# zju3dv/Mirror-NeRF

Hardware: AMD Instinct MI355X
Metric: rendered rays/sec (primary+reflected) (higher is better)
Workload: dtype f32 carried as hi/lo f16 pairs (f16 MFMA, f32 accumulate; max |diff| to the fp32 chain 3e-6)

## Files before the change

include/mnrf.h:

```cpp
#ifndef MNRF_H
#define MNRF_H

#include <stdint.h>

#ifdef __cplusplus
extern "C" {
#endif

#define MNRF_OK 0
#define MNRF_ERR_ARG (-1)
#define MNRF_ERR_LAUNCH (-2)
#define MNRF_ERR_UNSUPPORTED (-3)

#define MNRF_N_PARAMS 32

#define MNRF_SIGMA_ONLY 1u
#define MNRF_GRAD_NORMAL 2u
#define MNRF_SPLIT_F16 4u

#define MNRF_TCNN_GRAD_F16 16u
#define MNRF_TCNN_GRAD_FIXED 512u
#define MNRF_TCNN_F16 256u
#define MNRF_TCNN_TABLE_F16 1024u
#define MNRF_TCNN_VALU 8u
// ... 6 lines not shown

#define MNRF_GUARD_SATURATED 1u
#define MNRF_GUARD_WEIGHT 2u
#define MNRF_GUARD_IN_FORWARD 128u
#define MNRF_GUARD_IN_BACKWARD 256u
#define MNRF_GUARD_IN_SECOND_ORDER 512u
#define MNRF_GUARD_ENC_RANGE 4u

const char* mnrf_last_error(void);
int mnrf_version(void);

int64_t mnrf_packed_floats(void);

int mnrf_pack_weights(const float* const* params, float* packed, void* stream);
int mnrf_pack_weights_n(int n_models, const float* const* params, float* const* packed, void* stream);

int mnrf_embed(const float* x, int64_t n, int c, int n_freqs, float* out, void* stream);

int mnrf_field_forward(float* packed, unsigned flags, int64_t B,
                       const float* xyz, int64_t xyz_stride,
                       const float* rays, const float* z_vals, int spr,
                       const float* dir_emb, int64_t dir_stride,
                       float* sigma, float* rgb, float* pred_normal, float* is_mirror,
                       float* normal, float* geo_feat, void* stream);

int mnrf_sample_coarse(const float* rays, int64_t n_rays, const float* z_steps, int n_samples,
                       int use_disp, float perturb, const float* perturb_rand, float* z_vals,
                       void* stream);

int mnrf_composite(const float* rays, int64_t n_rays, int S, const float* sigma, const float* z_vals,
// ... 308 lines not shown
```

mirror_nerf_amd/_lib.py:

```python
import ctypes
import os
import subprocess

import torch

_HERE = os.path.dirname(os.path.abspath(__file__))
LIB_PATH = os.environ.get("MNRF_LIB", os.path.join(_HERE, "libmnrf_hip.so"))
CSRC = os.path.join(_HERE, "csrc")

_c_f = ctypes.c_void_p
_c_i = ctypes.c_void_p
_i64 = ctypes.c_int64
_int = ctypes.c_int
_u32 = ctypes.c_uint
_flt = ctypes.c_float
_str = ctypes.c_void_p

MNRF_SIGMA_ONLY = 1
MNRF_GRAD_NORMAL = 2
MNRF_SPLIT_F16 = 4
MNRF_TCNN_VALU = 8
MNRF_TCNN_F16 = 256
MNRF_TCNN_GRAD_FIXED = 512
MNRF_TCNN_TABLE_F16 = 1024
# ... 1 lines not shown
MNRF_CUT_MIRROR_HEAD = 64
MNRF_DW_ACCUMULATE = 128
MNRF_TRAIN_PLANES = 256
MNRF_PLANES_Y_HALF = 0x100000
MNRF_TCNN_GRAD_F16 = 16
MNRF_DETACH_W_MASK = 1
MNRF_DETACH_W_NORMAL = 2
N_PARAMS = 32

SIGNATURES = {
    "mnrf_last_error": (ctypes.c_char_p, []),
    "mnrf_version": (_int, []),
    "mnrf_packed_floats": (_i64, []),
    "mnrf_pack_weights": (_int, [ctypes.POINTER(ctypes.c_void_p), _c_f, _str]),
    "mnrf_pack_weights_n": (_int, [_int, ctypes.POINTER(ctypes.c_void_p), ctypes.POINTER(ctypes.c_void_p), _str]),
    "mnrf_embed": (_int, [_c_f, _i64, _int, _int, _c_f, _str]),
    "mnrf_field_forward": (_int, [_c_f, _u32, _i64, _c_f, _i64, _c_f, _c_f, _int, _c_f, _i64,
                                  _c_f, _c_f, _c_f, _c_f, _c_f, _c_f, _str]),
    "mnrf_sample_coarse": (_int, [_c_f, _i64, _c_f, _int, _int, _flt, _c_f, _c_f, _str]),
    "mnrf_composite": (_int, [_c_f, _i64, _int, _c_f, _c_f, _c_f, _c_f, _c_f, _c_f, _c_f, _int,
                              _c_f, _c_f, _c_f, _c_f, _c_f, _c_f, _c_f, _c_f, _c_f, _str]),
    "mnrf_composite_backward": (_int, [_c_f, _i64, _int] + [_c_f] * 7 + [_int] + [_c_f] * 17 + [_int, _c_f, _str]),
    "mnrf_reflect_backward": (_int, [_c_f, _c_f, _c_i, _i64, _c_f, _i64, _c_f, _c_f, _c_f, _str]),
    "mnrf_blend_backward": (_int, [_c_f, _c_f, _c_i, _i64, _i64, _int, _c_f, _c_f, _str]),
    "mnrf_embed_backward": (_int, [_c_f, _c_f, _i64, _int, _int, _c_f, _str]),
    "mnrf_ray_grads": (_int, [_c_f, _c_f, _c_f, _i64, _int, _c_f, _c_f, _str]),
    "mnrf_train_save_floats": (_i64, [_i64]),
    "mnrf_train_mask_words": (_i64, [_i64]),
    "mnrf_train_workspace_floats": (_i64, [_i64]),
    "mnrf_field_forward_train": (_int, [_c_f, _i64, _c_f, _i64, _c_f, _c_f, _int, _c_f, _i64] + [_c_f] * 9 + [_u32, _str]),
# ... 147 lines not shown
```

mirror_nerf_amd/csrc/mnrf_field.hip:

```cpp
#include <hip/hip_runtime.h>
#include <stdint.h>
#include <stdlib.h>

#include "mnrf_layout.h"
#include "mnrf_field_args.h"

namespace mnrf {

extern __shared__ __attribute__((aligned(16))) char smem[];

namespace s2 {
constexpr int S = 2;
constexpr int MIN_WAVES_PER_SIMD = 1;
constexpr int CHUNK_TILES = 16;
#include "mnrf_field_impl.inc"
#include "mnrf_field_bwd.inc"
}
namespace s1 {
constexpr int S = 1;
constexpr int MIN_WAVES_PER_SIMD = 2;
constexpr int CHUNK_TILES = 16;
#include "mnrf_field_impl.inc"
}

// ... 98 lines not shown
        const int nb = n_models - m0 < PACK_BATCH ? n_models - m0 : PACK_BATCH;
        PackBatch PB{};
        float* images[PACK_BATCH] = {};
        for (int m = 0; m < nb; ++m) {
            for (int i = 0; i < MNRF_N_PARAMS; ++i) PB.m[m].params[i] = params[(m0 + m) * MNRF_N_PARAMS + i];
            PB.m[m].packed = images[m] = packed[m0 + m];
        }
        hipLaunchKernelGGL(pack_kernel, dim3(blocks, nb), dim3(threads), 0, (hipStream_t)stream, PB, T);
        launch_split_pack(images, nb, (hipStream_t)stream);
        if (split32_enabled())
            for (int m = 0; m < nb; ++m) launch_split32_pack(params + (m0 + m) * MNRF_N_PARAMS, images[m], (hipStream_t)stream);
    }
    return mnrf_check_launch("mnrf_pack_weights");
}

extern "C" int mnrf_pack_weights(const float* const* params, float* packed, void* stream) {
    if (!params || !packed) return mnrf_fail(MNRF_ERR_ARG, "mnrf_pack_weights: null pointer");
    return mnrf_pack_weights_n(1, params, &packed, stream);
}

extern "C" int mnrf_field_forward(float* packed, unsigned flags, int64_t B, const float* xyz,
                                  int64_t xyz_stride, const float* rays, const float* z_vals, int spr,
                                  const float* dir_emb, int64_t dir_stride, float* sigma, float* rgb,
                                  float* pred_normal, float* is_mirror, float* normal, float* geo_feat,
                                  void* stream) {
    if (!packed) return mnrf_fail(MNRF_ERR_ARG, "mnrf_field_forward: packed weights are null");
    if (B < 0) return mnrf_fail(MNRF_ERR_ARG, "mnrf_field_forward: negative sample count");
    if (B == 0) return MNRF_OK;
    const bool sigma_only = flags & MNRF_SIGMA_ONLY;
    const bool grad = flags & MNRF_GRAD_NORMAL;
// ... 3 lines not shown
    if (!xyz && B % spr != 0) return mnrf_fail(MNRF_ERR_ARG, "mnrf_field_forward: B not a multiple of spr");
    if (!sigma_only && !dir_emb) return mnrf_fail(MNRF_ERR_ARG, "mnrf_field_forward: dir_emb required unless SIGMA_ONLY");
    if (grad && !normal) return mnrf_fail(MNRF_ERR_ARG, "mnrf_field_forward: GRAD_NORMAL needs the normal output");
    FieldArgs A{packed, flags, (long long)B, xyz, (long long)xyz_stride, rays, z_vals, spr, dir_emb,
                (long long)dir_stride, sigma, rgb, pred_normal, is_mirror, normal, geo_feat};
    static const int forced = [] {
        const char* e = getenv("MNRF_FIELD_VARIANT");
        if (e && e[0] == 's' && (e[1] == '1' || e[1] == '2')) return e[1] - '0';
        if (e && e[0] == 'h') return e[1] == 'x' ? 5 : (e[1] == '2' ? 4 : 3);
        return 0;
    }();
    const int variant = forced ? forced : ((flags & MNRF_SPLIT_F16) ? 3 + (int)((flags >> 3) & 3u) : (grad ? 1 : 2));
    const int rc = variant >= 3 ? launch_split(A, sigma_only, grad, variant - 3, (hipStream_t)stream)
                 : variant == 1 ? s1::launch(A, sigma_only, grad, (hipStream_t)stream)
                                : s2::launch(A, sigma_only, grad, (hipStream_t)stream);
    if (rc != 0) return mnrf_fail(MNRF_ERR_ARG, "mnrf_field_forward: too many samples for one launch");
    return mnrf_check_launch("mnrf_field_forward");
}

extern "C" int mnrf_fused_samples_per_ray(void) { return split48_ray_samples(); }

extern "C" int mnrf_field_composite_fused(float* packed, int64_t n_rays, const float* rays, const float* z_vals,
                                          const float* dir_emb, int64_t dir_stride, int white_back,
                                          float* weights, float* opacity, float* rgb_map, float* depth, float* mirror_mask,
                                          float* surf_normal, float* x_surface, void* stream) {
    if (!packed || !rays || !z_vals || !dir_emb) return mnrf_fail(MNRF_ERR_ARG, "mnrf_field_composite_fused: null pointer");
    if (n_rays < 0) return mnrf_fail(MNRF_ERR_ARG, "mnrf_field_composite_fused: negative ray count");
    if (n_rays == 0) return MNRF_OK;
    if (!split48_enabled() || split32_enabled())
        return mnrf_fail(MNRF_ERR_UNSUPPORTED, "mnrf_field_composite_fused: needs the 48-samples-per-wave tuning (MNRF_SPLIT48 != 0, MNRF_SPLIT32 unset)");
// ... 273 lines not shown
```

mirror_nerf_amd/csrc/mnrf_field_args.h:

```cpp
#pragma once
#include <hip/hip_runtime.h>
#include <stdint.h>

#include "../../include/mnrf.h"
#include "mnrf_layout.h"
#include "mnrf_dwp.h"

namespace mnrf {

typedef float f32x4 __attribute__((ext_vector_type(4)));

struct FieldArgs {
    const float* packed;
    unsigned flags;
    long long B;
    const float* xyz;
    long long xyz_stride;
    const float* rays;
    const float* z_vals;
    int spr;
    const float* dir_emb;
    long long dir_stride;
    float* sigma;
    float* rgb;
// ... 40 lines not shown
    const float* xyz; long long xyz_stride; const float* rays; const float* z_vals; int spr;
    const float* g_normal;
    const float* normal;
    const float* save_invj;
    const unsigned long long* save_mask;
    float* so;
    float* d_xyz;
    char* x2_planes;
    char* y2_planes;
    const unsigned* jmax;
    const int* n_live;
};

int launch_split(const FieldArgs& A, bool sigma_only, bool grad, int variant, hipStream_t s);
void launch_split_pack(float* const* packed, int n_images, hipStream_t s);
int launch_split_bwd(const FieldBwdArgs& A, hipStream_t s);
bool split48_enabled();
int launch_split48(const FieldArgs& A, bool sigma_only, hipStream_t s);
int split48_ray_samples();
bool split32_enabled();
int launch_split32(const FieldArgs& A, bool sigma_only, hipStream_t s);
void launch_split32_pack(const float* const* params, float* packed, hipStream_t s);
int launch_split_bwd2(const FieldBwd2Args& A, hipStream_t s);

}
```

mirror_nerf_amd/csrc/mnrf_field_split.hip:

```cpp
#include <hip/hip_runtime.h>
#include <stdint.h>
#include <type_traits>
#include <stdlib.h>

#include "mnrf_layout.h"
#include "mnrf_field_args.h"

namespace mnrf {

extern __shared__ __attribute__((aligned(16))) char smem[];

namespace h2 {
constexpr int S = 2;
constexpr int MIN_WAVES_PER_SIMD = 1;
constexpr int CHUNK_PAIRS = 8;
constexpr int RING_SLOTS = 4;
#include "mnrf_field_split.inc"
}
namespace h2x {
constexpr int S = 2;
constexpr int MIN_WAVES_PER_SIMD = 1;
constexpr int CHUNK_PAIRS = 16;
constexpr int RING_SLOTS = 3;
#include "mnrf_field_split.inc"
// ... 4 lines not shown
constexpr int S = 1;
constexpr int MIN_WAVES_PER_SIMD = 2;
constexpr int CHUNK_PAIRS = 8;
constexpr int RING_SLOTS = 3;
#define MNRF_SPLIT_NO_GRAD
#include "mnrf_field_split.inc"
#undef MNRF_SPLIT_NO_GRAD
}
#endif

int launch_split(const FieldArgs& A, bool sigma_only, bool grad, int variant, hipStream_t s) {
#ifdef MNRF_EXP_H1
    if (variant == 3 && !grad) return h1::launch(A, sigma_only, grad, s);
#endif
    if (!grad && variant == 0 && split32_enabled()) return launch_split32(A, sigma_only, s);
    if (!grad && variant == 0 && !A.geo_feat && split48_enabled()) return launch_split48(A, sigma_only, s);
    const bool big = variant == 0 ? grad : variant == 2;
    return big ? h2x::launch(A, sigma_only, grad, s) : h2::launch(A, sigma_only, grad, s);
}

int launch_split_bwd(const FieldBwdArgs& A, hipStream_t s) { return h2x::launch_bwd(A, s); }
int launch_split_bwd2(const FieldBwd2Args& A, hipStream_t s) { return h2x::launch_bwd2(A, s); }

struct SplitPackImages {
    float* packed[4];
};
__global__ void split_pack_kernel(SplitPackImages I, PartTable T) {
    float* packed = I.packed[blockIdx.y];
    const long long q = (long long)blockIdx.x * blockDim.x + threadIdx.x;
    constexpr long long FWD_LANES = (long long)SPLIT_FWD_PAIRS * 64;
// ... 52 lines not shown
    if (bad) atomicOr((unsigned*)(packed + PACKED_FLOATS - 1), MNRF_GUARD_WEIGHT);
    char* dst = (char*)(packed + (region == 2 ? OFF_SPLIT_HBWD : (region == 1 ? OFF_SPLIT_BWD : OFF_SPLIT_FWD))) + (long long)pair * PAIR_BYTES + lane * 16;
    *(h8v*)dst = hi;
    *(h8v*)(dst + PAIR_BYTES / 2) = lo;
}

void launch_split_pack(float* const* packed, int n_images, hipStream_t s) {
    PartTable T;
    build_parts(T);
    SplitPackImages I{};
    for (int m = 0; m < n_images; ++m) I.packed[m] = packed[m];
    const long long n = (long long)(SPLIT_FWD_PAIRS + SPLIT_BWD_PAIRS + SPLIT_HBWD_PAIRS) * 64;
    hipLaunchKernelGGL(split_pack_kernel, dim3((unsigned)((n + 255) / 256), n_images), dim3(256), 0, s, I, T);
}

}
```

mirror_nerf_amd/csrc/mnrf_field_split.inc:

```
constexpr int CHUNK_BYTES = CHUNK_PAIRS * PAIR_BYTES;
constexpr int WAVES = 4;
constexpr int WG_THREADS = 64 * WAVES;
constexpr int WG_SAMPLES = WAVES * S * 16;
constexpr int PIECES = CHUNK_BYTES / TILE_BYTES / WAVES;
constexpr int U = 2;
constexpr int PF = S == 3 ? 2 : 4;
constexpr int NBUF = PF + U;
typedef unsigned u32x4 __attribute__((ext_vector_type(4)));
typedef unsigned u32x2 __attribute__((ext_vector_type(2)));
typedef _Float16 h2v __attribute__((ext_vector_type(2)));
struct StoreCtx {
    __amdgpu_buffer_rsrc_t rsrc;
    __amdgpu_buffer_rsrc_t rsrc_lo;
    char* base;
    int lane;
    int soff;
    h2v fac[S];
};
__device__ __forceinline__ __amdgpu_buffer_rsrc_t plane_rsrc(char* sample_block) {
    return __builtin_amdgcn_make_buffer_rsrc(sample_block, 0, 0x7fffffff, 0x00020000);
}
static_assert(CHUNK_PAIRS / U == PIECES, "one LDS-DMA piece per wave per unit");
constexpr int LDS_RING = RING_SLOTS * CHUNK_BYTES;
constexpr int LDS_BIAS = LDS_RING;
// ... 418 lines not shown
            lo[s][nb >> 1][2 * (nb & 1) + 1] = l1;
        }
        if (WANT_MASK) ((uint64_t*)(smem + LDS_MASK))[(layer * S + s) * WG_THREADS + tid] = m;
    }
    sat_flush(sat, tmax);
}

__device__ __forceinline__ float sigmoidf_(float x) { return 1.f / (1.f + expf(-x)); }



template <bool SIGMA_ONLY, bool GRAD, bool PLANES = false, bool FUSE = false>
__global__ __launch_bounds__(WG_THREADS, MIN_WAVES_PER_SIMD) void field_split_kernel(FieldArgs A) {
    static_assert(!PLANES || (GRAD && !SIGMA_ONLY && S == 2), "operand planes: the training forward (32 samples per wave)");
    static_assert(!FUSE || (S == 3 && !SIGMA_ONLY && !GRAD), "ray-fused compositing: the 192-sample fine pass");
    float* const fz = (float*)(smem + LDS_FUSE);
    constexpr bool PERSIST = S == 3;
    if constexpr (PLANES) {
        if (A.n_live) {
            long long bl = (long long)*A.n_live * A.spr;
            bl = bl < 0 ? 0 : bl;
            if (bl < A.B) A.B = bl;
        }
        if ((long long)blockIdx.x * WG_SAMPLES >= A.B) return;
    }
    const bool queued = PERSIST && A.tile_queue != nullptr;
    const int wave = __builtin_amdgcn_readfirstlane(threadIdx.x >> 6);
    int tile = blockIdx.x;
    int round = 0;
    unsigned long long sat_all = 0, enc_all = 0;
    {
        const f32x4* src = (const f32x4*)(A.packed + OFF_BIAS);
        f32x4* dst = (f32x4*)(smem + LDS_BIAS);
        for (int i = threadIdx.x; i < BIAS_FLOATS / 4; i += WG_THREADS) dst[i] = src[i];
    }
    for (;;) {
    int lane_;
    if (PERSIST) asm volatile("v_mbcnt_lo_u32_b32 %0, -1, 0\n\tv_mbcnt_hi_u32_b32 %0, -1, %0" : "=v"(lane_));
    else lane_ = threadIdx.x & 63;
    const int lane = lane_;
    const int tid = PERSIST ? wave * 64 + lane : (int)threadIdx.x;
    const int g = lane >> 4;
    const int m = lane & 15;
    const int lane16 = lane * 16;
    constexpr int HP = (S == 3 && !SIGMA_ONLY && !GRAD) ? HEAD_PARK : 0;
    char* const pl = (PLANES || (GRAD && S == 2 && A.save_planes))
                         ? A.save_planes + ((long long)blockIdx.x * WAVES + wave) * PLX_SB_BYTES : nullptr;
// ... 15 lines not shown
    sc.soff = 0;
    const auto at_h = [&](int sec, int T0) -> const StoreCtx& {
        sc.soff = (SEC_H / 16 + 16 * sec + 2 * T0) * PL_FB_BYTES;
        return sc;
    };
#ifdef MNRF_EXP_CYCLES
#define MNRF_MARK(k) do { if (tid == 0 && A.geo_feat) ((long long*)A.geo_feat)[tile * 16 + (k)] = (long long)__builtin_amdgcn_s_memtime(); } while (0)
#else
#define MNRF_MARK(k) do { } while (0)
#endif
    MNRF_MARK(0);

    Stream st;
    st.sat = 0;
    st.tmax = 0.f;
    open_stream<true>(st, A.packed + OFF_SPLIT_FWD, wave, lane);
    int next_tile = 0;
    if (queued && tid == 0) next_tile = (int)gridDim.x + atomicAdd(A.tile_queue, 1);

    int idx[S];
    bool valid[S];
#pragma unroll
    for (int s = 0; s < S; ++s) {
        long long i = (long long)tile * WG_SAMPLES + wave * (S * 16) + s * 16 + m;
        valid[s] = i < A.B;
        if (!valid[s]) i = A.B - 1;
        idx[s] = (int)i;
    }
    const auto m15 = [&]() -> unsigned {
        unsigned r;
        asm volatile("v_mbcnt_lo_u32_b32 %0, -1, 0\n\tv_mbcnt_hi_u32_b32 %0, -1, %0\n\tv_and_b32 %0, 15, %0" : "=v"(r));
// ... 194 lines not shown
#pragma unroll
            for (int s = 0; s < S; ++s) {
                if (valid[s]) {
                    f32x4* o = (f32x4*)(A.geo_feat + (long long)idx[s] * 256);
#pragma unroll
                    for (int nb = 0; nb < 16; ++nb) {
                        const f32x4 v = nb < 8 ? accA[s][nb & 7] : accB[s][nb & 7];
                        o[nb * 4 + g] = f32x4{fmaxf(v[0], 0.f), fmaxf(v[1], 0.f), fmaxf(v[2], 0.f), fmaxf(v[3], 0.f)};
                    }
                }
            }
        }
#endif
    }
    MNRF_MARK(5);
    {
        f32x4 acc[S][1];
        init_bias<1>(acc, BIAS_SIG, gq());
        gemm_part<8, 1, 960, HP>(acc, hh, hl, st, wave, lane16);
        if (FUSE) {
            if (gq() == 0) {
#pragma unroll
                for (int s = 0; s < S; ++s) fz[wave * (S * 16) + s * 16 + m15()] = acc[s][0][0];
            }
        } else if (A.sigma && g == 0) {
#pragma unroll
            for (int s = 0; s < S; ++s)
                if (sval(s)) out_store(A.sigma + sidx(s), acc[s][0][0]);
        }
    }

    MNRF_MARK(6);
    if (!SIGMA_ONLY) {
        {
            u32x4 nh[S][4], nl[S][4];
            {
                f32x4 acc[S][8];
                init_bias<8>(acc, BIAS_NRM1, gq());
                gemm_part<8, 8, 968, HP, ST0>(acc, hh, hl, st, wave, lane16, at_h(7, 0));
                if (keep) save_acc<8, 0>(A.save_x + (long long)SEC_HN * A.B, 128, 0, acc, idx, valid, g, unused_bits);
                acc_to_b<8, 0, false>(nh, nl, acc, 0, tid, st.sat);
                if constexpr (S == 2) { if (pl) store_planes<4, 4>(sc, SEC_HN / 16, nh, nl); }
            }
            f32x4 acc[S][1];
            init_bias<1>(acc, BIAS_NRM2, gq());
            gemm_part<4, 1, 1032>(acc, nh, nl, st, wave, lane16);
            if (FUSE) {
                if (gq() == 0) {
#pragma unroll
                    for (int s = 0; s < S; ++s) {
                        const float a0 = acc[s][0][0], a1 = acc[s][0][1], a2 = acc[s][0][2];
                        const float inv = 1.f / sqrtf(fmaxf(a0 * a0 + a1 * a1 + a2 * a2, 1.1920928955078125e-07f));
                        const int q = wave * (S * 16) + s * 16 + (int)m15();
                        fz[4 * WG_SAMPLES + q] = a0 * inv; fz[5 * WG_SAMPLES + q] = a1 * inv; fz[6 * WG_SAMPLES + q] = a2 * inv;
                    }
                }
            } else if (A.pred_normal && g == 0) {
#pragma unroll
                for (int s = 0; s < S; ++s)
                    if (sval(s)) {
                        const float a0 = acc[s][0][0], a1 = acc[s][0][1], a2 = acc[s][0][2];
                        const float inv = 1.f / sqrtf(fmaxf(a0 * a0 + a1 * a1 + a2 * a2, 1.1920928955078125e-07f));
                        float* o = A.pred_normal + (long long)sidx(s) * 3;
                        out_store(o, a0 * inv); out_store(o + 1, a1 * inv); out_store(o + 2, a2 * inv);
                        if (GRAD && A.save_inv)
                            A.save_inv[idx[s]] = (a0 * a0 + a1 * a1 + a2 * a2) > 1.1920928955078125e-07f ? inv : -inv;
                    }
            }
        }
        MNRF_MARK(7);
        {
            u32x4 mh[S][4], ml[S][4];
            {
                f32x4 acc[S][8];
                init_bias<8>(acc, BIAS_MIR1, gq());
                gemm_part<8, 8, 1036, HP, ST4>(acc, hh, hl, st, wave, lane16, at_h(7, 4));
                if (keep) {
                    uint64_t bits[S];
                    save_acc<8, 2>(A.save_x + (long long)SEC_HM * A.B, 128, 0, acc, idx, valid, g, bits);
#pragma unroll
                    for (int s = 0; s < S; ++s) gmask[(9 * S + s) * WG_THREADS + tid] = bits[s];
                } else if (GRAD && pl) {
                    store_sign_mask<8>(acc, gmask + (9 * S) * WG_THREADS + tid);
                }
                acc_to_b<8, 2, false>(mh, ml, acc, 0, tid, st.sat);
                if constexpr (S == 2) { if (pl) store_planes<4, 4>(sc, SEC_HM / 16, mh, ml); }
            }
            f32x4 acc[S][1];
            init_bias<1>(acc, BIAS_MIR2, gq());
            gemm_part<4, 1, 1100>(acc, mh, ml, st, wave, lane16);
            if (FUSE) {
                if (gq() == 0) {
#pragma unroll
                    for (int s = 0; s < S; ++s) fz[7 * WG_SAMPLES + wave * (S * 16) + s * 16 + m15()] = sigmoidf_(acc[s][0][0]);
                }
            } else if (A.is_mirror && g == 0) {
#pragma unroll
                for (int s = 0; s < S; ++s)
                    if (sval(s)) out_store(A.is_mirror + sidx(s), sigmoidf_(acc[s][0][0]));
            }
        }
        MNRF_MARK(8);
        {
            u32x4 dh[S][4], dl[S][4];
            {
                u32x4 fh[S][8], fl[S][8];
                {
                    f32x4 acc[S][16];
                    init_bias<16>(acc, BIAS_FIN, gq());
                    gemm_part<8, 16, 1104, HP>(acc, hh, hl, st, wave, lane16);
                    if (keep) save_acc<16, 0>(A.save_x + (long long)SEC_FIN * A.B, 256, 0, acc, idx, valid, g, unused_bits);
                    acc_to_b<16, 0, false>(fh, fl, acc, 0, tid, st.sat);
                    if constexpr (S == 2) { if (pl) store_planes<8, 8>(sc, SEC_FIN / 16, fh, fl); }
                }
                u32x4 vh[S][1], vl[S][1];
                {
                    float de[S][8];
                    const int gv = gq();
                    const int spr = opaque_spr();
#pragma unroll
                    for (int s = 0; s < S; ++s) {
                        const float* dp = A.dir_emb + (long long)(sidx(s) / spr) * A.dir_stride;
#pragma unroll
                        for (int t = 0; t < 8; ++t) {
                            const int e = 16 * (t >> 2) + 4 * gv + (t & 3);
                            de[s][t] = e < ENC_DIR ? dp[e] : 0.f;
                        }
                    }
                    if (keep) save_bform<8>(A.save_x + (long long)SEC_DIRE * A.B, 32, de, idx, valid, g);
                    split_b<8>(de, vh, vl, st.sat);
                    if constexpr (S == 2) { if (pl) store_planes<1, 1>(sc, SEC_DIRE / 16, vh, vl); }
                }
                MNRF_MARK(9);
                f32x4 acc[S][8];
                init_bias<8>(acc, BIAS_DIR, gq());
                gemm_part<8, 8, 1232>(acc, fh, fl, st, wave, lane16);
                gemm_part<1, 8, 1296>(acc, vh, vl, st, wave, lane16);
                if (keep) {
                    uint64_t bits[S];
                    save_acc<8, 1>(A.save_x + (long long)SEC_HD * A.B, 128, 0, acc, idx, valid, g, bits);
#pragma unroll
                    for (int s = 0; s < S; ++s) gmask[(8 * S + s) * WG_THREADS + tid] = bits[s];
                } else if (GRAD && pl) {
                    store_sign_mask<8>(acc, gmask + (8 * S) * WG_THREADS + tid);
                }
                acc_to_b<8, 1, false>(dh, dl, acc, 0, tid, st.sat);
                if constexpr (S == 2) { if (pl) store_planes<4, 4>(sc, SEC_HD / 16, dh, dl); }
            }
            f32x4 acc[S][1];
            init_bias<1>(acc, BIAS_RGB, gq());
            gemm_part<4, 1, 1304>(acc, dh, dl, st, wave, lane16);
            if (FUSE) {
                if (gq() == 0) {
#pragma unroll
                    for (int s = 0; s < S; ++s) {
                        const int q = wave * (S * 16) + s * 16 + (int)m15();
                        fz[1 * WG_SAMPLES + q] = sigmoidf_(acc[s][0][0]);
                        fz[2 * WG_SAMPLES + q] = sigmoidf_(acc[s][0][1]);
                        fz[3 * WG_SAMPLES + q] = sigmoidf_(acc[s][0][2]);
                    }
                }
            } else if (A.rgb && g == 0) {
#pragma unroll
                for (int s = 0; s < S; ++s)
                    if (sval(s)) {
                        float* o = A.rgb + (long long)sidx(s) * 3;
// ... 160 lines not shown
```

mirror_nerf_amd/csrc/mnrf_layout.h:

```cpp
#pragma once
#include <stdint.h>

namespace mnrf {

constexpr int W = 256;
constexpr int ENC_XYZ = 63;
constexpr int ENC_DIR = 27;
constexpr int NFREQ_XYZ = 10;
constexpr int NFREQ_DIR = 4;

constexpr int TILE_FLOATS = 256;
constexpr int TILE_BYTES = 1024;
constexpr int PAD_TILES = 16;

enum PartKind : int {
    KIND_H = 0,
    KIND_ENC = 1,
    KIND_DIR = 2,
};

__host__ __device__ inline int enc_col(int t, int g) {
    const int P = 8 * g + (t >> 1);
    const int s = t & 1;
    if (P < 30) return 3 + 6 * (P / 3) + 3 * s + (P % 3);
// ... 53 lines not shown
constexpr int64_t OFF_SPLIT_BWD = OFF_SPLIT_FWD + (int64_t)SPLIT_FWD_PAIRS * (PAIR_BYTES / 4);
constexpr int64_t OFF_SPLIT_HBWD = OFF_SPLIT_BWD + (int64_t)SPLIT_BWD_PAIRS * (PAIR_BYTES / 4);
constexpr int SPLIT32_FWD_USED_SIGMA = 960 + 16;
constexpr int SPLIT32_FWD_USED = SPLIT32_FWD_USED_SIGMA + 64 + 8 + 64 + 8 + 128 + 64 + 8 + 8;
constexpr int SPLIT32_FWD_PAIRS = padded_pairs(SPLIT32_FWD_USED);
constexpr int64_t OFF_SPLIT32_FWD = OFF_SPLIT_HBWD + (int64_t)SPLIT_HBWD_PAIRS * (PAIR_BYTES / 4);
__host__ __device__ inline int enc_col32(int T, int h, int e) {
    const int P = 16 * h + 4 * T + (e >> 1);
    const int s = e & 1;
    if (P < 30) return 3 + 6 * (P / 3) + 3 * s + (P % 3);
    if (P == 30) return s;
    return s == 0 ? 2 : -1;
}
constexpr int64_t SPLIT_TAIL_FLOATS = 2 * 16 * (PAIR_BYTES / 4);
constexpr int64_t PACKED_FLOATS = OFF_SPLIT32_FWD + (int64_t)SPLIT32_FWD_PAIRS * (PAIR_BYTES / 4) + SPLIT_TAIL_FLOATS;
constexpr int TQ_PAIRS = 8;
constexpr int64_t OFF_TILE_QUEUE = PACKED_FLOATS - 1 - 2 * TQ_PAIRS;
constexpr int64_t OFF_REDUCE_PAIR = OFF_TILE_QUEUE - 2;
constexpr int DEVICE_STATE_WORDS = 2 + 2 * TQ_PAIRS + 1;

constexpr int SEC_ENC = 0;
constexpr int SEC_H = 64;
constexpr int SEC_FIN = 2112;
constexpr int SEC_DIRE = 2368;
constexpr int SEC_HD = 2400;
constexpr int SEC_HN = 2528;
constexpr int SEC_HM = 2656;
constexpr int SAVE_FLOATS = 2784;
constexpr int N_MASKS = 10;
constexpr int DY_L = 0;
constexpr int DY_FIN = 2048;
constexpr int DY_DIR = 2304;
constexpr int DY_NRM1 = 2432;
constexpr int DY_MIR1 = 2560;
// ... 61 lines not shown
```

mirror_nerf_amd/mirror_nerf.py:

```python
import os

import torch
from torch import nn

from . import _lib
from .weights import packed_of


class Embedding(nn.Module):

    def __init__(self, N_freqs, logscale=True):
        super().__init__()
        if not logscale:
            raise NotImplementedError("only logscale=True (the reference default) is implemented")
        self.N_freqs = N_freqs
        self.freq_bands = 2 ** torch.linspace(0, N_freqs - 1, N_freqs) if N_freqs > 0 else torch.zeros(0)

    def forward(self, x):
        x = x.float().contiguous()
        n, c = x.shape
        out = torch.empty(n, c * (2 * self.N_freqs + 1), dtype=torch.float32, device=x.device)
        if n:
            _lib.check(_lib.lib().mnrf_embed(_lib.ptr(x), n, c, self.N_freqs, _lib.ptr(out), _lib.stream()),
                       "mnrf_embed")
# ... 170 lines not shown
        if old_pin is not None:
            module.__dict__["_mnrf_precision"] = old_pin
    return {k: float((out["fp32"][k] - out["split"][k]).abs().max() / max(1.0, float(out["fp32"][k].abs().max())))
            for k in out["fp32"]}


LAUNCH_LOG = None

FLOP_FULL = 1318912
FLOP_SIGMA = 982528
FLOP_GRAD = 982528


def field_forward(module, B, *, xyz=None, xyz_stride=3, rays=None, z_vals=None, spr=1, dir_emb=None,
                  dir_stride=27, sigma_only=False, grad_normal=False, want_geo=False, device=None):
    packed = packed_of(module)
    dev = packed.device
    f = lambda *s: torch.empty(*s, dtype=torch.float32, device=dev)
    out = {"sigma": f(B)}
    if getattr(module, "predict_normal", True) and not sigma_only:
        out["pred_normal"] = f(B, 3)
    if not sigma_only:
        out["rgb"] = f(B, 3)
        if getattr(module, "predict_mirror_mask", True):
            out["is_mirror"] = f(B)
    if grad_normal:
        out["normal"] = f(B, 3)
    if want_geo:
        out["geo_feat"] = f(B, 256)
    flags = (_lib.MNRF_SIGMA_ONLY if sigma_only else 0) | (_lib.MNRF_GRAD_NORMAL if grad_normal else 0)
    prec = precision_of(module)
# ... 106 lines not shown
```

mirror_nerf_amd/rendering.py:

```python
import torch

from . import _lib
from .autograd import CompositeFn, EmbedFn, FieldFn
from .mirror_nerf import field_forward
from .weights import params_of

__all__ = ["render_rays", "sample_pdf"]

_LINSPACE = {}


def _linspace01(n, device):
    key = (n, str(device))
    t = _LINSPACE.get(key)
    if t is None:
        t = torch.linspace(0, 1, n).to(device)
        _LINSPACE[key] = t
    return t


def _n_freqs(emb):
    n = getattr(emb, "N_freqs", None)
    if n is None:
        raise RuntimeError("embeddings must expose N_freqs (Embedding modules)")
# ... 112 lines not shown
        from .autograd import RayFanFn
        r_cf, r_ff, r_cc, r_fc, de_c, de_f, z_vals = RayFanFn.apply(rays, n_fd, z_steps, N_samples, bool(use_disp), float(perturb),
                                                                   prand, n_live)
        per_pass = {"_noise_coarse": (r_fc, r_cc, de_c), "_noise_fine": (r_ff, r_cf, de_f)}
    else:
        z_vals = f(N, N_samples)
        if N:
            _lib.check(L.mnrf_sample_coarse_n(p(rays), N, p(z_steps), N_samples, int(bool(use_disp)), float(perturb),
                                              p(prand), p(z_vals), p(n_live), _lib.stream()), "mnrf_sample_coarse")

    has_fine = "fine" in models
    results = {}

    def inference_fused(model, typ, z):
        from . import mirror_nerf as _mn
        from .weights import packed_of
        if _mn.precision_of(model) != "split" or z.shape[1] != L.mnrf_fused_samples_per_ray():
            return False
        has_m, has_n = getattr(model, "predict_mirror_mask", True), getattr(model, "predict_normal", True)
        opacity, rgb_map, depth, xs = f(N), f(N, 3), f(N), f(N, 3)
        mask = f(N) if has_m else None
        sn = f(N, 3) if has_n else None
        if _mn.LAUNCH_LOG is not None:
            e0, e1 = torch.cuda.Event(enable_timing=True), torch.cuda.Event(enable_timing=True)
            e0.record()
        rc = L.mnrf_field_composite_fused(p(packed_of(model)), N, p(rays), p(z), p(dir_emb), dir_emb.shape[1], int(bool(white_back)),
                                          None, p(opacity), p(rgb_map), p(depth), p(mask), p(sn), p(xs), _lib.stream())
        if rc == -3:
            return False
        _lib.check(rc, "mnrf_field_composite_fused")
        if _mn.LAUNCH_LOG is not None:
            e1.record()
            _mn.LAUNCH_LOG.append((_lib.MNRF_SPLIT_F16 | 0x2000, N * z.shape[1], e0, e1))
        results[f"opacity_{typ}"] = opacity
        results[f"z_vals_{typ}"] = z
        results[f"rgb_{typ}"] = rgb_map
        results[f"depth_{typ}"] = depth
        if has_m:
            results[f"mirror_mask_{typ}"] = mask
        if has_n:
            results[f"surface_normal_{typ}"] = sn
# ... 174 lines not shown
```

mirror_nerf_amd/weights.py:

```python
import ctypes

import torch

from . import _lib

PARAM_NAMES = []
for _i in range(8):
    PARAM_NAMES += [f"xyz_encoding_{_i+1}.0.weight", f"xyz_encoding_{_i+1}.0.bias"]
PARAM_NAMES += ["xyz_encoding_final.weight", "xyz_encoding_final.bias",
                "dir_encoding.0.weight", "dir_encoding.0.bias",
                "sigma.weight", "sigma.bias", "rgb.0.weight", "rgb.0.bias",
                "normal_net.0.weight", "normal_net.0.bias", "normal_net.1.weight", "normal_net.1.bias",
                "is_mirror_net.0.weight", "is_mirror_net.0.bias", "is_mirror_net.2.weight", "is_mirror_net.2.bias"]

PARAM_SHAPES = {}
for _i in range(8):
    _in = 63 if _i == 0 else (319 if _i == 4 else 256)
    PARAM_SHAPES[f"xyz_encoding_{_i+1}.0.weight"] = (256, _in)
    PARAM_SHAPES[f"xyz_encoding_{_i+1}.0.bias"] = (256,)
PARAM_SHAPES.update({
    "xyz_encoding_final.weight": (256, 256), "xyz_encoding_final.bias": (256,),
    "dir_encoding.0.weight": (128, 283), "dir_encoding.0.bias": (128,),
    "sigma.weight": (1, 256), "sigma.bias": (1,), "rgb.0.weight": (3, 128), "rgb.0.bias": (3,),
    "normal_net.0.weight": (128, 256), "normal_net.0.bias": (128,),
# ... 97 lines not shown
    _GENERATION[0] += 1


try:
    from torch.optim.optimizer import register_optimizer_step_post_hook as _reg_hook
    _reg_hook(bump_generation)
except ImportError:
    _reg_hook = None


class PackedCache:

    def __init__(self):
        self.key = None
        self.packed = None

    def stale(self, module):
        refs = param_refs(module)
        key = [_GENERATION[0]]
        for sub, pname, _ in refs:
            q = sub._parameters[pname]
            key.append(q.data_ptr())
            key.append(q._version)
        if _reg_hook is None and any(sub._parameters[pname].requires_grad for sub, pname, _ in refs):
            self.key = None
        return key if (key != self.key or self.packed is None) else None

    def get(self, module):
        key = self.stale(module)
        if key is not None:
            self.packed = pack_state({full: sub._parameters[pname] for sub, pname, full in param_refs(module)}, self.packed)
            self.key = key
        return self.packed


def packed_of_many(modules):
    caches, todo = [], []
    for m in modules:
        cache = m.__dict__.get("_mnrf_packed")
        if cache is None:
            cache = m.__dict__["_mnrf_packed"] = PackedCache()
        caches.append(cache)
        key = cache.stale(m)
        if key is not None:
            todo.append((m, cache, key))
    if len({next(iter(m.parameters())).device for m, _, _ in todo}) > 1:
        return [c.get(m) for m, c in zip(modules, caches)]
    if todo:
        outs = pack_states([{full: sub._parameters[pname] for sub, pname, full in param_refs(m)} for m, _, _ in todo],
                           [c.packed for _, c, _ in todo])
        for (m, c, key), out in zip(todo, outs):
            c.packed, c.key = out, key
    return [c.packed for c in caches]


def invalidate_packed(module):
    cache = module.__dict__.get("_mnrf_packed")
    if cache is not None:
        cache.key = None
    if hasattr(module, "_blob_key"):
        module._blob_key = None


_VALIDATED = {}


class validated:
# ... 11 lines not shown
    def __exit__(self, *exc):
        for k in self.added:
            _VALIDATED.pop(k, None)
        return False


def packed_of(module):
    hit = _VALIDATED.get(id(module))
    if hit is not None:
        return hit
    cache = module.__dict__.get("_mnrf_packed")
    if cache is None:
        cache = PackedCache()
        module.__dict__["_mnrf_packed"] = cache
    return cache.get(module)
```

Before: 1.636 million.

## Fold normal and view-direction linear layers into preceding layers for inference

Adds a weight-folding pass that precomputes products of consecutive linear layers with no activation between them (normal head second layer times first layer, direction layer times the feature layer) in double precision. It stores the result as a separate hi/lo f16 pair stream and bias block inside the packed image. The inference forward then skips the intermediate normal-hidden and final-feature GEMMs, feeding the hidden state straight into the folded weights. This removes two GEMM stages per sample, at the cost of a one-time fold per weight update. It also changes rounding slightly, and the fold is disabled when the split32 path is on.

After: 1.852 million (median of 6 runs). 13.2% higher.

```diff
diff --git a/include/mnrf.h b/include/mnrf.h
--- a/include/mnrf.h
+++ b/include/mnrf.h
@@ -44,6 +44,7 @@
 
 int mnrf_pack_weights(const float* const* params, float* packed, void* stream);
 int mnrf_pack_weights_n(int n_models, const float* const* params, float* const* packed, void* stream);
+int mnrf_fold_weights_n(int n_models, const float* const* params, float* const* packed, void* stream);
 
 int mnrf_embed(const float* x, int64_t n, int c, int n_freqs, float* out, void* stream);
 
diff --git a/mirror_nerf_amd/_lib.py b/mirror_nerf_amd/_lib.py
--- a/mirror_nerf_amd/_lib.py
+++ b/mirror_nerf_amd/_lib.py
@@ -39,6 +39,7 @@
     "mnrf_packed_floats": (_i64, []),
     "mnrf_pack_weights": (_int, [ctypes.POINTER(ctypes.c_void_p), _c_f, _str]),
     "mnrf_pack_weights_n": (_int, [_int, ctypes.POINTER(ctypes.c_void_p), ctypes.POINTER(ctypes.c_void_p), _str]),
+    "mnrf_fold_weights_n": (_int, [_int, ctypes.POINTER(ctypes.c_void_p), ctypes.POINTER(ctypes.c_void_p), _str]),
     "mnrf_embed": (_int, [_c_f, _i64, _int, _int, _c_f, _str]),
     "mnrf_field_forward": (_int, [_c_f, _u32, _i64, _c_f, _i64, _c_f, _c_f, _int, _c_f, _i64,
                                   _c_f, _c_f, _c_f, _c_f, _c_f, _c_f, _str]),
diff --git a/mirror_nerf_amd/csrc/mnrf_field.hip b/mirror_nerf_amd/csrc/mnrf_field.hip
--- a/mirror_nerf_amd/csrc/mnrf_field.hip
+++ b/mirror_nerf_amd/csrc/mnrf_field.hip
@@ -136,6 +136,21 @@
     return mnrf_check_launch("mnrf_pack_weights");
 }
 
+extern "C" int mnrf_fold_weights_n(int n_models, const float* const* params, float* const* packed, void* stream) {
+    if (n_models < 0) return mnrf_fail(MNRF_ERR_ARG, "mnrf_fold_weights_n: negative model count");
+    if (n_models == 0 || split32_enabled()) return MNRF_OK;
+    if (!params || !packed) return mnrf_fail(MNRF_ERR_ARG, "mnrf_fold_weights_n: null pointer");
+    for (int i = 0; i < n_models * MNRF_N_PARAMS; ++i)
+        if (!params[i]) return mnrf_fail(MNRF_ERR_ARG, "mnrf_fold_weights_n: null parameter pointer");
+    for (int m = 0; m < n_models; ++m)
+        if (!packed[m]) return mnrf_fail(MNRF_ERR_ARG, "mnrf_fold_weights_n: null image pointer");
+    for (int m0 = 0; m0 < n_models; m0 += PACK_BATCH) {
+        const int nb = n_models - m0 < PACK_BATCH ? n_models - m0 : PACK_BATCH;
+        launch_split_fold(params + m0 * MNRF_N_PARAMS, packed + m0, nb, (hipStream_t)stream);
+    }
+    return mnrf_check_launch("mnrf_fold_weights");
+}
+
 extern "C" int mnrf_pack_weights(const float* const* params, float* packed, void* stream) {
     if (!params || !packed) return mnrf_fail(MNRF_ERR_ARG, "mnrf_pack_weights: null pointer");
     return mnrf_pack_weights_n(1, params, &packed, stream);
@@ -169,6 +184,7 @@
     const int rc = variant >= 3 ? launch_split(A, sigma_only, grad, variant - 3, (hipStream_t)stream)
                  : variant == 1 ? s1::launch(A, sigma_only, grad, (hipStream_t)stream)
                                 : s2::launch(A, sigma_only, grad, (hipStream_t)stream);
+    if (rc == -2) return mnrf_fail(MNRF_ERR_UNSUPPORTED, "mnrf_field_forward: a forced h2 / hx forward variant needs the folded stream (MNRF_SPLIT32 unset)");
     if (rc != 0) return mnrf_fail(MNRF_ERR_ARG, "mnrf_field_forward: too many samples for one launch");
     return mnrf_check_launch("mnrf_field_forward");
 }
diff --git a/mirror_nerf_amd/csrc/mnrf_field_args.h b/mirror_nerf_amd/csrc/mnrf_field_args.h
--- a/mirror_nerf_amd/csrc/mnrf_field_args.h
+++ b/mirror_nerf_amd/csrc/mnrf_field_args.h
@@ -78,6 +78,7 @@
 
 int launch_split(const FieldArgs& A, bool sigma_only, bool grad, int variant, hipStream_t s);
 void launch_split_pack(float* const* packed, int n_images, hipStream_t s);
+void launch_split_fold(const float* const* params, float* const* packed, int n_images, hipStream_t s);
 int launch_split_bwd(const FieldBwdArgs& A, hipStream_t s);
 bool split48_enabled();
 int launch_split48(const FieldArgs& A, bool sigma_only, hipStream_t s);
diff --git a/mirror_nerf_amd/csrc/mnrf_field_split.hip b/mirror_nerf_amd/csrc/mnrf_field_split.hip
--- a/mirror_nerf_amd/csrc/mnrf_field_split.hip
+++ b/mirror_nerf_amd/csrc/mnrf_field_split.hip
@@ -42,6 +42,7 @@
     if (variant == 3 && !grad) return h1::launch(A, sigma_only, grad, s);
 #endif
     if (!grad && variant == 0 && split32_enabled()) return launch_split32(A, sigma_only, s);
+    if (!grad && !sigma_only && split32_enabled()) return -2;
     if (!grad && variant == 0 && !A.geo_feat && split48_enabled()) return launch_split48(A, sigma_only, s);
     const bool big = variant == 0 ? grad : variant == 2;
     return big ? h2x::launch(A, sigma_only, grad, s) : h2::launch(A, sigma_only, grad, s);
@@ -124,4 +125,94 @@
     hipLaunchKernelGGL(split_pack_kernel, dim3((unsigned)((n + 255) / 256), n_images), dim3(256), 0, s, I, T);
 }
 
-}
+struct FoldImages {
+    float* packed[4];
+    const float* wfin[4];
+    const float* wdir[4];
+    const float* wn1[4];
+    const float* wn2[4];
+};
+__global__ void split_fold_kernel(FoldImages I) {
+    float* packed = I.packed[blockIdx.y];
+    const long long q = (long long)blockIdx.x * blockDim.x + threadIdx.x;
+    constexpr long long FOLD_LANES = (long long)SPLIT_FOLD_PAIRS * 64;
+    if (q >= FOLD_LANES + BIAS_FLOATS) return;
+    const float* bias = packed + OFF_BIAS;
+    if (q >= FOLD_LANES) {
+        const int b = (int)(q - FOLD_LANES);
+        float v = bias[b];
+        if (b > BIAS_SIG && b <= BIAS_SIG + 3) {
+            const int i = b - BIAS_SIG - 1;
+            const float* w2 = I.wn2[blockIdx.y] + i * 128;
+            double a = 0.0;
+            for (int k = 0; k < 128; ++k) a = fma((double)w2[k], (double)bias[BIAS_NRM1 + k], a);
+            v = (float)(a + (double)bias[BIAS_NRM2 + i]);
+        } else if (b >= BIAS_DIR && b < BIAS_DIR + 128) {
+            const float* wd = I.wdir[blockIdx.y] + (b - BIAS_DIR) * (W + ENC_DIR);
+            double a = 0.0;
+            for (int k = 0; k < W; ++k) a = fma((double)wd[k], (double)bias[BIAS_FIN + k], a);
+            v = (float)(a + (double)bias[b]);
+        }
+        packed[OFF_FOLD_BIAS + b] = v;
+        return;
+    }
+    const int pair = (int)(q >> 6);
+    const int lane = (int)(q & 63);
+    const int row = lane & 15;
+    typedef _Float16 h8v __attribute__((ext_vector_type(8)));
+    h8v hi, lo;
+    for (int j = 0; j < 8; ++j) hi[j] = lo[j] = (_Float16)0.f;
+    const int sp = pair < 968 ? pair : (pair < 1036 ? pair + (1036 - 968) : (pair >= 1100 && pair < 1112 ? pair + (1296 - 1100) : -1));
+    if (sp >= 0) {
+        const char* src = (const char*)(packed + OFF_SPLIT_FWD) + (long long)sp * PAIR_BYTES + lane * 16;
+        hi = *(const h8v*)src;
+        lo = *(const h8v*)(src + PAIR_BYTES / 2);
+    }
+    const bool fold_nrm = pair >= 960 && pair < 968 && row >= 1 && row <= 3;
+    const bool fold_dir = pair >= 1036 && pair < 1100;
+    if (fold_nrm || fold_dir) {
+        const int T = fold_nrm ? pair - 960 : (pair - 1036) / 8;
+        const int c0 = 32 * T + 4 * (lane >> 4);
+        const float* a = fold_nrm ? I.wn2[blockIdx.y] + (row - 1) * 128 : I.wdir[blockIdx.y] + (16 * ((pair - 1036) % 8) + row) * (W + ENC_DIR);
+        const float* bm = fold_nrm ? I.wn1[blockIdx.y] : I.wfin[blockIdx.y];
+        const int K = fold_nrm ? 128 : W;
+        double acc[8];
+        for (int j = 0; j < 8; ++j) acc[j] = 0.0;
+        for (int k = 0; k < K; ++k) {
+            const double ak = (double)a[k];
+            const float* bk = bm + (long long)k * W + c0;
+#pragma unroll
+            for (int c = 0; c < 4; ++c) {
+                acc[c] = fma(ak, (double)bk[c], acc[c]);
+                acc[4 + c] = fma(ak, (double)bk[16 + c], acc[4 + c]);
+            }
+        }
+        bool bad = false;
+#pragma unroll
+        for (int j = 0; j < 8; ++j) {
+            hi[j] = (_Float16)acc[j];
+            lo[j] = (_Float16)(acc[j] - (double)hi[j]);
+            bad |= !(fabs(acc[j]) < 65504.0);
+        }
+        if (bad) atomicOr((unsigned*)(packed + PACKED_FLOATS - 1), MNRF_GUARD_WEIGHT);
+    }
+    char* dst = (char*)(packed + OFF_FOLD_FWD) + (long long)pair * PAIR_BYTES + lane * 16;
+    *(h8v*)dst = hi;
+    *(h8v*)(dst + PAIR_BYTES / 2) = lo;
+}
+
+void launch_split_fold(const float* const* params, float* const* packed, int n_images, hipStream_t s) {
+    FoldImages I{};
+    for (int m = 0; m < n_images; ++m) {
+        const float* const* p = params + m * 32;
+        I.packed[m] = packed[m];
+        I.wfin[m] = p[16];
+        I.wdir[m] = p[18];
+        I.wn1[m] = p[24];
+        I.wn2[m] = p[26];
+    }
+    const long long n = (long long)SPLIT_FOLD_PAIRS * 64 + BIAS_FLOATS;
+    hipLaunchKernelGGL(split_fold_kernel, dim3((unsigned)((n + 255) / 256), n_images), dim3(256), 0, s, I);
+}
+
+}
diff --git a/mirror_nerf_amd/csrc/mnrf_field_split.inc b/mirror_nerf_amd/csrc/mnrf_field_split.inc
--- a/mirror_nerf_amd/csrc/mnrf_field_split.inc
+++ b/mirror_nerf_amd/csrc/mnrf_field_split.inc
@@ -456,6 +456,7 @@
 __global__ __launch_bounds__(WG_THREADS, MIN_WAVES_PER_SIMD) void field_split_kernel(FieldArgs A) {
     static_assert(!PLANES || (GRAD && !SIGMA_ONLY && S == 2), "operand planes: the training forward (32 samples per wave)");
     static_assert(!FUSE || (S == 3 && !SIGMA_ONLY && !GRAD), "ray-fused compositing: the 192-sample fine pass");
+    constexpr bool FOLD = !SIGMA_ONLY && !GRAD;
     float* const fz = (float*)(smem + LDS_FUSE);
     constexpr bool PERSIST = S == 3;
     if constexpr (PLANES) {
@@ -472,7 +473,7 @@
     int round = 0;
     unsigned long long sat_all = 0, enc_all = 0;
     {
-        const f32x4* src = (const f32x4*)(A.packed + OFF_BIAS);
+        const f32x4* src = (const f32x4*)(A.packed + (FOLD ? OFF_FOLD_BIAS : OFF_BIAS));
         f32x4* dst = (f32x4*)(smem + LDS_BIAS);
         for (int i = threadIdx.x; i < BIAS_FLOATS / 4; i += WG_THREADS) dst[i] = src[i];
     }
@@ -518,7 +519,7 @@
     Stream st;
     st.sat = 0;
     st.tmax = 0.f;
-    open_stream<true>(st, A.packed + OFF_SPLIT_FWD, wave, lane);
+    open_stream<true>(st, A.packed + (FOLD ? OFF_FOLD_FWD : OFF_SPLIT_FWD), wave, lane);
     int next_tile = 0;
     if (queued && tid == 0) next_tile = (int)gridDim.x + atomicAdd(A.tile_queue, 1);
 
@@ -743,6 +744,31 @@
 #endif
     }
     MNRF_MARK(5);
+    const auto put_normal = [&](const f32x4 (&acc)[S][1], auto r0) {
+        constexpr int R0 = decltype(r0)::value;
+        if (FUSE) {
+            if (gq() == 0) {
+#pragma unroll
+                for (int s = 0; s < S; ++s) {
+                    const float a0 = acc[s][0][R0], a1 = acc[s][0][R0 + 1], a2 = acc[s][0][R0 + 2];
+                    const float inv = 1.f / sqrtf(fmaxf(a0 * a0 + a1 * a1 + a2 * a2, 1.1920928955078125e-07f));
+                    const int q = wave * (S * 16) + s * 16 + (int)m15();
+                    fz[4 * WG_SAMPLES + q] = a0 * inv; fz[5 * WG_SAMPLES + q] = a1 * inv; fz[6 * WG_SAMPLES + q] = a2 * inv;
+                }
+            }
+        } else if (A.pred_normal && g == 0) {
+#pragma unroll
+            for (int s = 0; s < S; ++s)
+                if (sval(s)) {
+                    const float a0 = acc[s][0][R0], a1 = acc[s][0][R0 + 1], a2 = acc[s][0][R0 + 2];
+                    const float inv = 1.f / sqrtf(fmaxf(a0 * a0 + a1 * a1 + a2 * a2, 1.1920928955078125e-07f));
+                    float* o = A.pred_normal + (long long)sidx(s) * 3;
+                    out_store(o, a0 * inv); out_store(o + 1, a1 * inv); out_store(o + 2, a2 * inv);
+                    if (GRAD && A.save_inv)
+                        A.save_inv[idx[s]] = (a0 * a0 + a1 * a1 + a2 * a2) > 1.1920928955078125e-07f ? inv : -inv;
+                }
+        }
+    };
     {
         f32x4 acc[S][1];
         init_bias<1>(acc, BIAS_SIG, gq());
@@ -757,11 +783,12 @@
             for (int s = 0; s < S; ++s)
                 if (sval(s)) out_store(A.sigma + sidx(s), acc[s][0][0]);
         }
+        if constexpr (FOLD) put_normal(acc, std::integral_constant<int, 1>{});
     }
 
     MNRF_MARK(6);
     if (!SIGMA_ONLY) {
-        {
+        if constexpr (!FOLD) {
             u32x4 nh[S][4], nl[S][4];
             {
                 f32x4 acc[S][8];
@@ -774,28 +801,7 @@
             f32x4 acc[S][1];
             init_bias<1>(acc, BIAS_NRM2, gq());
             gemm_part<4, 1, 1032>(acc, nh, nl, st, wave, lane16);
-            if (FUSE) {
-                if (gq() == 0) {
-#pragma unroll
-                    for (int s = 0; s < S; ++s) {
-                        const float a0 = acc[s][0][0], a1 = acc[s][0][1], a2 = acc[s][0][2];
-                        const float inv = 1.f / sqrtf(fmaxf(a0 * a0 + a1 * a1 + a2 * a2, 1.1920928955078125e-07f));
-                        const int q = wave * (S * 16) + s * 16 + (int)m15();
-                        fz[4 * WG_SAMPLES + q] = a0 * inv; fz[5 * WG_SAMPLES + q] = a1 * inv; fz[6 * WG_SAMPLES + q] = a2 * inv;
-                    }
-                }
-            } else if (A.pred_normal && g == 0) {
-#pragma unroll
-                for (int s = 0; s < S; ++s)
-                    if (sval(s)) {
-                        const float a0 = acc[s][0][0], a1 = acc[s][0][1], a2 = acc[s][0][2];
-                        const float inv = 1.f / sqrtf(fmaxf(a0 * a0 + a1 * a1 + a2 * a2, 1.1920928955078125e-07f));
-                        float* o = A.pred_normal + (long long)sidx(s) * 3;
-                        out_store(o, a0 * inv); out_store(o + 1, a1 * inv); out_store(o + 2, a2 * inv);
-                        if (GRAD && A.save_inv)
-                            A.save_inv[idx[s]] = (a0 * a0 + a1 * a1 + a2 * a2) > 1.1920928955078125e-07f ? inv : -inv;
-                    }
-            }
+            put_normal(acc, std::integral_constant<int, 0>{});
         }
         MNRF_MARK(7);
         {
@@ -803,7 +809,7 @@
             {
                 f32x4 acc[S][8];
                 init_bias<8>(acc, BIAS_MIR1, gq());
-                gemm_part<8, 8, 1036, HP, ST4>(acc, hh, hl, st, wave, lane16, at_h(7, 4));
+                gemm_part<8, 8, FOLD ? 968 : 1036, HP, ST4>(acc, hh, hl, st, wave, lane16, at_h(7, 4));
                 if (keep) {
                     uint64_t bits[S];
                     save_acc<8, 2>(A.save_x + (long long)SEC_HM * A.B, 128, 0, acc, idx, valid, g, bits);
@@ -817,7 +823,7 @@
             }
             f32x4 acc[S][1];
             init_bias<1>(acc, BIAS_MIR2, gq());
-            gemm_part<4, 1, 1100>(acc, mh, ml, st, wave, lane16);
+            gemm_part<4, 1, FOLD ? 1032 : 1100>(acc, mh, ml, st, wave, lane16);
             if (FUSE) {
                 if (gq() == 0) {
 #pragma unroll
@@ -830,9 +836,35 @@
             }
         }
         MNRF_MARK(8);
+        const auto view_operands = [&](u32x4 (&vh)[S][1], u32x4 (&vl)[S][1]) {
+            float de[S][8];
+            const int gv = gq();
+            const int spr = opaque_spr();
+#pragma unroll
+            for (int s = 0; s < S; ++s) {
+                const float* dp = A.dir_emb + (long long)(sidx(s) / spr) * A.dir_stride;
+#pragma unroll
+                for (int t = 0; t < 8; ++t) {
+                    const int e = 16 * (t >> 2) + 4 * gv + (t & 3);
+                    de[s][t] = e < ENC_DIR ? dp[e] : 0.f;
+                }
+            }
+            if (keep) save_bform<8>(A.save_x + (long long)SEC_DIRE * A.B, 32, de, idx, valid, g);
+            split_b<8>(de, vh, vl, st.sat);
+            if constexpr (S == 2) { if (pl) store_planes<1, 1>(sc, SEC_DIRE / 16, vh, vl); }
+        };
         {
             u32x4 dh[S][4], dl[S][4];
-            {
+            if constexpr (FOLD) {
+                u32x4 vh[S][1], vl[S][1];
+                view_operands(vh, vl);
+                MNRF_MARK(9);
+                f32x4 acc[S][8];
+                init_bias<8>(acc, BIAS_DIR, gq());
+                gemm_part<8, 8, 1036, HP>(acc, hh, hl, st, wave, lane16);
+                gemm_part<1, 8, 1100>(acc, vh, vl, st, wave, lane16);
+                acc_to_b<8, 1, false>(dh, dl, acc, 0, tid, st.sat);
+            } else {
                 u32x4 fh[S][8], fl[S][8];
                 {
                     f32x4 acc[S][16];
@@ -843,23 +875,7 @@
                     if constexpr (S == 2) { if (pl) store_planes<8, 8>(sc, SEC_FIN / 16, fh, fl); }
                 }
                 u32x4 vh[S][1], vl[S][1];
-                {
-                    float de[S][8];
-                    const int gv = gq();
-                    const int spr = opaque_spr();
-#pragma unroll
-                    for (int s = 0; s < S; ++s) {
-                        const float* dp = A.dir_emb + (long long)(sidx(s) / spr) * A.dir_stride;
-#pragma unroll
-                        for (int t = 0; t < 8; ++t) {
-                            const int e = 16 * (t >> 2) + 4 * gv + (t & 3);
-                            de[s][t] = e < ENC_DIR ? dp[e] : 0.f;
-                        }
-                    }
-                    if (keep) save_bform<8>(A.save_x + (long long)SEC_DIRE * A.B, 32, de, idx, valid, g);
-                    split_b<8>(de, vh, vl, st.sat);
-                    if constexpr (S == 2) { if (pl) store_planes<1, 1>(sc, SEC_DIRE / 16, vh, vl); }
-                }
+                view_operands(vh, vl);
                 MNRF_MARK(9);
                 f32x4 acc[S][8];
                 init_bias<8>(acc, BIAS_DIR, gq());
@@ -878,7 +894,7 @@
             }
             f32x4 acc[S][1];
             init_bias<1>(acc, BIAS_RGB, gq());
-            gemm_part<4, 1, 1304>(acc, dh, dl, st, wave, lane16);
+            gemm_part<4, 1, FOLD ? 1108 : 1304>(acc, dh, dl, st, wave, lane16);
             if (FUSE) {
                 if (gq() == 0) {
 #pragma unroll
diff --git a/mirror_nerf_amd/csrc/mnrf_layout.h b/mirror_nerf_amd/csrc/mnrf_layout.h
--- a/mirror_nerf_amd/csrc/mnrf_layout.h
+++ b/mirror_nerf_amd/csrc/mnrf_layout.h
@@ -91,10 +91,15 @@
 }
 constexpr int64_t SPLIT_TAIL_FLOATS = 2 * 16 * (PAIR_BYTES / 4);
 constexpr int64_t PACKED_FLOATS = OFF_SPLIT32_FWD + (int64_t)SPLIT32_FWD_PAIRS * (PAIR_BYTES / 4) + SPLIT_TAIL_FLOATS;
+constexpr int SPLIT_FOLD_USED = 960 + 8 + 64 + 4 + 64 + 8 + 4;
+constexpr int SPLIT_FOLD_PAIRS = padded_pairs(SPLIT_FOLD_USED);
+constexpr int64_t OFF_FOLD_FWD = OFF_SPLIT32_FWD;
+constexpr int64_t OFF_FOLD_BIAS = OFF_FOLD_FWD + (int64_t)SPLIT_FOLD_PAIRS * (PAIR_BYTES / 4) + SPLIT_TAIL_FLOATS;
 constexpr int TQ_PAIRS = 8;
 constexpr int64_t OFF_TILE_QUEUE = PACKED_FLOATS - 1 - 2 * TQ_PAIRS;
 constexpr int64_t OFF_REDUCE_PAIR = OFF_TILE_QUEUE - 2;
 constexpr int DEVICE_STATE_WORDS = 2 + 2 * TQ_PAIRS + 1;
+static_assert(OFF_FOLD_BIAS + BIAS_FLOATS <= OFF_REDUCE_PAIR, "the folded stream and its bias block fit the 32x32x16 region");
 
 constexpr int SEC_ENC = 0;
 constexpr int SEC_H = 64;
diff --git a/mirror_nerf_amd/mirror_nerf.py b/mirror_nerf_amd/mirror_nerf.py
--- a/mirror_nerf_amd/mirror_nerf.py
+++ b/mirror_nerf_amd/mirror_nerf.py
@@ -4,7 +4,7 @@
 from torch import nn
 
 from . import _lib
-from .weights import packed_of
+from .weights import folded_of, packed_of
 
 
 class Embedding(nn.Module):
@@ -208,7 +208,7 @@
 
 def field_forward(module, B, *, xyz=None, xyz_stride=3, rays=None, z_vals=None, spr=1, dir_emb=None,
                   dir_stride=27, sigma_only=False, grad_normal=False, want_geo=False, device=None):
-    packed = packed_of(module)
+    packed = folded_of(module) if precision_of(module).startswith("split") and not sigma_only and not grad_normal else packed_of(module)
     dev = packed.device
     f = lambda *s: torch.empty(*s, dtype=torch.float32, device=dev)
     out = {"sigma": f(B)}
diff --git a/mirror_nerf_amd/rendering.py b/mirror_nerf_amd/rendering.py
--- a/mirror_nerf_amd/rendering.py
+++ b/mirror_nerf_amd/rendering.py
@@ -150,7 +150,7 @@
 
     def inference_fused(model, typ, z):
         from . import mirror_nerf as _mn
-        from .weights import packed_of
+        from .weights import folded_of
         if _mn.precision_of(model) != "split" or z.shape[1] != L.mnrf_fused_samples_per_ray():
             return False
         has_m, has_n = getattr(model, "predict_mirror_mask", True), getattr(model, "predict_normal", True)
@@ -160,7 +160,7 @@
         if _mn.LAUNCH_LOG is not None:
             e0, e1 = torch.cuda.Event(enable_timing=True), torch.cuda.Event(enable_timing=True)
             e0.record()
-        rc = L.mnrf_field_composite_fused(p(packed_of(model)), N, p(rays), p(z), p(dir_emb), dir_emb.shape[1], int(bool(white_back)),
+        rc = L.mnrf_field_composite_fused(p(folded_of(model)), N, p(rays), p(z), p(dir_emb), dir_emb.shape[1], int(bool(white_back)),
                                           None, p(opacity), p(rgb_map), p(depth), p(mask), p(sn), p(xs), _lib.stream())
         if rc == -3:
             return False
diff --git a/mirror_nerf_amd/weights.py b/mirror_nerf_amd/weights.py
--- a/mirror_nerf_amd/weights.py
+++ b/mirror_nerf_amd/weights.py
@@ -135,6 +135,7 @@
     def __init__(self):
         self.key = None
         self.packed = None
+        self.folded = False
 
     def stale(self, module):
         refs = param_refs(module)
@@ -152,7 +153,16 @@
         if key is not None:
             self.packed = pack_state({full: sub._parameters[pname] for sub, pname, full in param_refs(module)}, self.packed)
             self.key = key
+            self.folded = False
         return self.packed
+
+    def fold(self, module):
+        if not self.folded:
+            L = _lib.lib()
+            arr, img, keep = (ctypes.c_void_p * _lib.N_PARAMS)(), (ctypes.c_void_p * 1)(self.packed.data_ptr()), []
+            _param_pointers({full: sub._parameters[pname] for sub, pname, full in param_refs(module)}, arr, 0, keep)
+            _lib.check(L.mnrf_fold_weights_n(1, arr, img, _lib.stream()), "mnrf_fold_weights")
+            self.folded = True
 
 
 def packed_of_many(modules):
@@ -171,7 +181,7 @@
         outs = pack_states([{full: sub._parameters[pname] for sub, pname, full in param_refs(m)} for m, _, _ in todo],
                            [c.packed for _, c, _ in todo])
         for (m, c, key), out in zip(todo, outs):
-            c.packed, c.key = out, key
+            c.packed, c.key, c.folded = out, key, False
     return [c.packed for c in caches]
 
 
@@ -213,3 +223,12 @@
         cache = PackedCache()
         module.__dict__["_mnrf_packed"] = cache
     return cache.get(module)
+
+
+def folded_of(module):
+    image = packed_of(module)
+    cache = module.__dict__["_mnrf_packed"]
+    if cache.packed is not image:
+        raise RuntimeError("folded_of: the validated image is not the module's cached one")
+    cache.fold(module)
+    return image
```
